# selau642/QuantizedAttention

Measured on AMD Instinct MI355X. Metric: fused-attn fwd+bwd TFLOP/s & us/call at (B,H,S,D)=(4,32,4096,128), int8 vs bf16, higher is better.
Workload: dtype int8; 1 GPU; config 3: int8 SageAttention-3 fwd+bwd (4,32,4096,128) per rank, non-causal; global_batch=4, parallelism=batch x head shard over 1 GPU(s)

## Files before the change

### quantizedattention_amd/csrc/int8_bwd.hip

```cpp
#include <climits>
#include <type_traits>
#include <cstdlib>

#include "tile_image.h"

namespace qattn {

template <int D>
struct I8BwdCfg {
  static constexpr int NKS8 = D / 32;
  static constexpr int NDB = D / 32;
  static constexpr int T8 = I8Rows<D>::TILE;
  static constexpr int T16 = B16Tr<D>::TILE;
};

QA_DEVICE void quant_operand(const float* x, float inv, float c, v8bf* out) {
#pragma unroll
  for (int s = 0; s < 2; ++s) {
    v4u w;
#pragma unroll
    for (int j = 0; j < 4; ++j) {
      const int i0 = 8 * s + 2 * j;
      w[j] = pk_bf16(__builtin_truncf(x[i0] * inv) * c, __builtin_truncf(x[i0 + 1] * inv) * c);
    }
    out[s] = __builtin_bit_cast(v8bf, w);
  }
}

#ifndef QA_PREP_HOIST
#define QA_PREP_HOIST 1
#endif
template <int D, bool IMG>
__global__ __launch_bounds__(256) void int8_bwd_prep_kernel(
    const _Float16* __restrict__ dO, const _Float16* __restrict__ O, const _Float16* __restrict__ lse,
    int8_t* __restrict__ idx, _Float16* __restrict__ scale, __bf16* __restrict__ img,
    float2* __restrict__ LD, long nblocks) {
  constexpr int ELEMS = 32 * D;
  constexpr int ITERS = ELEMS / 512;
  constexpr int TPR = D / 8;
  const int lane = threadIdx.x & 63;
  const long blk = (long)blockIdx.x * 4 + (threadIdx.x >> 6);
  if (blk >= nblocks) return;
  const _Float16* xb = dO + blk * ELEMS;
  const _Float16* ob = O + blk * ELEMS;
  v8h v[ITERS];
  float amax = 0.f;
#if QA_PREP_HOIST
  v8h ov[ITERS];
  _Float16 lsev[ITERS];
#pragma unroll
  for (int i = 0; i < ITERS; ++i) {
    const int e = (i * 64 + lane) * 8;
    v[i] = *reinterpret_cast<const v8h*>(xb + e);
    ov[i] = *reinterpret_cast<const v8h*>(ob + e);
    lsev[i] = lse[blk * 32 + e / D];
  }
#endif
#pragma unroll
  for (int i = 0; i < ITERS; ++i) {
    const int e = (i * 64 + lane) * 8;
#if QA_PREP_HOIST
    const v8h o = ov[i];
#else
    v[i] = *reinterpret_cast<const v8h*>(xb + e);
    const v8h o = *reinterpret_cast<const v8h*>(ob + e);
#endif
    float dsum = 0.f;
#pragma unroll
    for (int j = 0; j < 8; ++j) {
      amax = fmaxf(amax, fabsf((float)v[i][j]));
      dsum += (float)(_Float16)((float)v[i][j] * (float)o[j]);
    }
#pragma unroll
    for (int m = TPR / 2; m >= 1; m >>= 1) dsum += __shfl_xor(dsum, m);
    if (lane % TPR == 0) {
      const long row = blk * 32 + e / D;
#if QA_PREP_HOIST
      LD[row] = float2{(float)lsev[i], (float)(_Float16)dsum};
#else
      LD[row] = float2{(float)lse[row], (float)(_Float16)dsum};
#endif
    }
  }
  amax = wave_max_f(amax);
  const _Float16 s16 = (_Float16)(amax / 127.0f);
  const float s = (float)s16;
  const float r = quant_rcp(s);
  if (lane == 0) scale[blk] = s16;
#pragma unroll
  for (int i = 0; i < ITERS; ++i) {
    const int e = (i * 64 + lane) * 8;
    unsigned lo, hi;
    float qf[8];
    quant8(v[i], s, r, lo, hi, qf);
    *reinterpret_cast<v2u*>(idx + blk * ELEMS + e) = v2u{lo, hi};
    if constexpr (IMG) {
      const v4u w = {pk_bf16(qf[0], qf[1]), pk_bf16(qf[2], qf[3]), pk_bf16(qf[4], qf[5]),
                     pk_bf16(qf[6], qf[7])};
      *reinterpret_cast<v4u*>(img + blk * ELEMS + e) = w;
    }
  }
}
__global__ __launch_bounds__(256) void i8_to_bf16_kernel(const int8_t* __restrict__ x,
                                                         __bf16* __restrict__ y, long n16) {
  const long i = (long)blockIdx.x * 256 + threadIdx.x;
  if (i >= n16) return;
  const v4i w = reinterpret_cast<const v4i*>(x)[i];
  v4u lo, hi;
#pragma unroll
  for (int k = 0; k < 4; ++k) {
    unsigned p[2];
#pragma unroll
    for (int j = 0; j < 2; ++j) {
      const float a = (float)((w[k] << (24 - 16 * j)) >> 24);
      const float b = (float)((w[k] << (16 - 16 * j)) >> 24);
      p[j] = (__float_as_uint(a) >> 16) | (__float_as_uint(b) & 0xffff0000u);
    }
    if (k < 2) { lo[2 * k] = p[0]; lo[2 * k + 1] = p[1]; }
    else { hi[2 * k - 4] = p[0]; hi[2 * k - 3] = p[1]; }
  }
  reinterpret_cast<v4u*>(y)[2 * i] = lo;
  reinterpret_cast<v4u*>(y)[2 * i + 1] = hi;
}

enum BwdRole { ROLE_DV = 0, ROLE_DK = 1, ROLE_DQ = 2, ROLE_DKV = 3 };
#ifndef QA_DKV_PIPE
#define QA_DKV_PIPE 0
#endif
#ifndef QA_DKV_STAGGER
#define QA_DKV_STAGGER 1
#endif
#ifndef QA_DKV_I8DV_COST
#define QA_DKV_I8DV_COST 0
#endif
#ifndef QA_DKV_WAVES
#define QA_DKV_WAVES 8
#endif
#ifndef QA_DKV_NSLOT
#define QA_DKV_NSLOT 4
#endif
#ifndef QA_DKV_HG
#define QA_DKV_HG 4
#endif
#ifndef QA_DQW_HG
#define QA_DQW_HG 0
#endif
#ifndef QA_DKV_PRIO
#define QA_DKV_PRIO 0
#endif
#ifndef QA_DQW_PRIO
#define QA_DQW_PRIO 0
#endif
#ifndef QA_BWD_PACK_ASM
#define QA_BWD_PACK_ASM 1
#endif


template <int D, int ROLE>
struct BwdCfg {
  using C = I8BwdCfg<D>;
  static constexpr bool TWO = ROLE != ROLE_DV;
  static constexpr bool HAS_LD = ROLE != ROLE_DQ;
  static constexpr bool WANT_P = ROLE == ROLE_DV || ROLE == ROLE_DKV;
  static constexpr bool WANT_DS = ROLE != ROLE_DV;
  static constexpr int NTR = (ROLE == ROLE_DKV) ? 2 : 1;
  static constexpr int WAVES = (ROLE == ROLE_DKV) ? QA_DKV_WAVES : 4;
  static constexpr bool PIPE = ROLE != ROLE_DKV;
  static constexpr int Y8A = 0;
  static constexpr int Y8B = C::T8;
  static constexpr int TR = TWO ? 2 * C::T8 : C::T8;
  static constexpr int TR2 = TR + C::T16;
  static constexpr int LDO = TR + NTR * C::T16;
  static constexpr int SLOT = LDO + (HAS_LD ? 256 : 0);
  static constexpr int NSLOT = (ROLE == ROLE_DKV) ? QA_DKV_NSLOT : 4;
  static constexpr int NP8 = I8Rows<D>::NP, NP16 = B16Tr<D>::NP;
  static constexpr int INST = NP8 * (TWO ? 2 : 1) + NTR * NP16;
  static constexpr int IPW16 = (INST + WAVES - 1) / WAVES;
  static constexpr int IPW = IPW16 + (HAS_LD ? 1 : 0);
  static constexpr int XROWS = 32 * WAVES;
};

template <int D, typename G>
struct BwdDmaT {
  unsigned voff[G::IPW16];
  unsigned lds_off[G::IPW16];
  unsigned stride[G::IPW16];
  v4u rsrc[G::IPW16];
  v4u ld_rsrc;
  QA_DEVICE void init(int wave, int lane, int S, const char* y8a, const char* y8b, const char* tr,
                      const char* tr2, const char* ld) {
#pragma unroll
    for (int i = 0; i < G::IPW16; ++i) {
      int p = wave + G::WAVES * i;
      if (p >= G::INST) p = wave;
      if (p < G::NP8) {
        set_i8(i, G::Y8A, p, lane);
        rsrc[i] = make_rsrc(y8a, (unsigned)S * D);
      } else if (G::TWO && p < 2 * G::NP8) {
        set_i8(i, G::Y8B, p - G::NP8, lane);
        rsrc[i] = make_rsrc(y8b, (unsigned)S * D);
      } else {
        int q = p - (G::TWO ? 2 : 1) * G::NP8;
        const bool second = q >= G::NP16;
        if (second) q -= G::NP16;
        voff[i] = B16Tr<D>::dma_src(q, lane);
        lds_off[i] = (second ? G::TR2 : G::TR) + q * 1024;
        stride[i] = B16Tr<D>::TILE;
        rsrc[i] = make_rsrc(second ? tr2 : tr, (unsigned)S * 2 * D);
      }
    }
    if constexpr (G::HAS_LD) ld_rsrc = make_rsrc(ld, (unsigned)S * 8);
  }
  QA_DEVICE void set_i8(int i, int region, int piece, int lane) {
    voff[i] = I8Rows<D>::dma_src(piece, lane);
    lds_off[i] = region + piece * 1024;
    stride[i] = I8Rows<D>::TILE;
  }
  QA_DEVICE void issue(unsigned slot_lds, int t, int lane) const {
#pragma unroll
    for (int i = 0; i < G::IPW16; ++i)
      dma16_buf(rsrc[i], voff[i], (unsigned)t * stride[i], slot_lds + lds_off[i]);
    if constexpr (G::HAS_LD) dma4_buf(ld_rsrc, 4 * lane, (unsigned)t * 256, slot_lds + G::LDO);
  }
};
template <int D, int ROLE>
using BwdDma = BwdDmaT<D, BwdCfg<D, ROLE>>;


QA_DEVICE void floor_magic16(float* y, float inv) {
  const float magic = 8388608.0f;
  asm("s_setreg_imm32_b32 hwreg(HW_REG_MODE, 0, 2), 3\n\t"
      "s_nop 1\n\t"
      "v_fma_f32 %0, %0, %16, %17\n\tv_fma_f32 %1, %1, %16, %17\n\t"
      "v_fma_f32 %2, %2, %16, %17\n\tv_fma_f32 %3, %3, %16, %17\n\t"
      "v_fma_f32 %4, %4, %16, %17\n\tv_fma_f32 %5, %5, %16, %17\n\t"
      "v_fma_f32 %6, %6, %16, %17\n\tv_fma_f32 %7, %7, %16, %17\n\t"
      "v_fma_f32 %8, %8, %16, %17\n\tv_fma_f32 %9, %9, %16, %17\n\t"
      "v_fma_f32 %10, %10, %16, %17\n\tv_fma_f32 %11, %11, %16, %17\n\t"
      "v_fma_f32 %12, %12, %16, %17\n\tv_fma_f32 %13, %13, %16, %17\n\t"
      "v_fma_f32 %14, %14, %16, %17\n\tv_fma_f32 %15, %15, %16, %17\n\t"
      "s_setreg_imm32_b32 hwreg(HW_REG_MODE, 0, 2), 0\n\t"
      "s_nop 1"
      : "+v"(y[0]), "+v"(y[1]), "+v"(y[2]), "+v"(y[3]), "+v"(y[4]), "+v"(y[5]), "+v"(y[6]),
        "+v"(y[7]), "+v"(y[8]), "+v"(y[9]), "+v"(y[10]), "+v"(y[11]), "+v"(y[12]), "+v"(y[13]),
        "+v"(y[14]), "+v"(y[15])
      : "v"(inv), "s"(magic));
}

QA_DEVICE v4i pack16_i8(const float* x) {
  float r0 = x[0], r1 = x[4], r2 = x[8], r3 = x[12];
#define QA_SDWA(R, A, B, U) \
  "v_cvt_i32_f32_sdwa " R ", " A " dst_sel:BYTE_" B " dst_unused:UNUSED_" U " src0_sel:DWORD\n\t"
  asm(QA_SDWA("%0", "%0", "0", "PAD") QA_SDWA("%1", "%1", "0", "PAD")
      QA_SDWA("%2", "%2", "0", "PAD") QA_SDWA("%3", "%3", "0", "PAD")
      QA_SDWA("%0", "%4", "1", "PRESERVE") QA_SDWA("%1", "%7", "1", "PRESERVE")
      QA_SDWA("%2", "%10", "1", "PRESERVE") QA_SDWA("%3", "%13", "1", "PRESERVE")
      QA_SDWA("%0", "%5", "2", "PRESERVE") QA_SDWA("%1", "%8", "2", "PRESERVE")
      QA_SDWA("%2", "%11", "2", "PRESERVE") QA_SDWA("%3", "%14", "2", "PRESERVE")
      QA_SDWA("%0", "%6", "3", "PRESERVE") QA_SDWA("%1", "%9", "3", "PRESERVE")
      QA_SDWA("%2", "%12", "3", "PRESERVE") QA_SDWA("%3", "%15", "3", "PRESERVE")
      : "+v"(r0), "+v"(r1), "+v"(r2), "+v"(r3)
      : "v"(x[1]), "v"(x[2]), "v"(x[3]), "v"(x[5]), "v"(x[6]), "v"(x[7]), "v"(x[9]), "v"(x[10]),
        "v"(x[11]), "v"(x[13]), "v"(x[14]), "v"(x[15]));
#undef QA_SDWA
  return v4i{__float_as_int(r0), __float_as_int(r1), __float_as_int(r2), __float_as_int(r3)};
}

QA_DEVICE float max16_abs3(const float* x) {
  float m = fmaxf(fmaxf(fabsf(x[0]), fabsf(x[1])), fabsf(x[2]));
#pragma unroll
  for (int i = 3; i < 15; i += 2) m = fmaxf(fmaxf(m, fabsf(x[i])), fabsf(x[i + 1]));
  return fmaxf(m, fabsf(x[15]));
}

template <int D>
QA_DEVICE void store_acc_row(const v16f* acc, float sc, _Float16* dst, const long& row, const int& h) {
#pragma unroll
  for (int b = 0; b < D / 32; ++b) {
#pragma unroll
    for (int g = 0; g < 4; ++g) {
      v4h w;
#pragma unroll
      for (int j = 0; j < 4; ++j) w[j] = (_Float16)(acc[b][4 * g + j] * sc);
      *reinterpret_cast<v4h*>(dst + row * D + 32 * b + 8 * g + 4 * h) = w;
    }
  }
}

#ifndef QA_DKV_STAMP
#define QA_DKV_STAMP 0
#endif
#if QA_DKV_STAMP
__device__ unsigned long long g_dkv_stamp[4096][4];
#define DKV_STAMP(k)                                                                            \
  do {                                                                                          \
    if (ROLE == ROLE_DKV && WS && threadIdx.x == 0 && blockIdx.x < 4096)                         \
      g_dkv_stamp[blockIdx.x][k] = __builtin_amdgcn_s_memrealtime();                            \
  } while (0)
#else
#define DKV_STAMP(k) do { } while (0)
#endif
template <int D, int ROLE, bool CAUSAL = false, bool WS = false>
__global__ __launch_bounds__((64 * BwdCfg<D, ROLE>::WAVES), (8 / BwdCfg<D, ROLE>::WAVES))
void int8_bwd_kernel(
    const int8_t* __restrict__ x8a, const int8_t* __restrict__ x8b, const _Float16* __restrict__ sxa,
    const _Float16* __restrict__ sxb, const int8_t* __restrict__ y8a, const int8_t* __restrict__ y8b,
    const __bf16* __restrict__ ytr, const __bf16* __restrict__ ytr2, const float2* __restrict__ yld,
    const _Float16* __restrict__ sya, const _Float16* __restrict__ syb,
    const float2* __restrict__ xld, _Float16* __restrict__ out, _Float16* __restrict__ out2, int BH,
    int Sx, int Ny, int ydiv, int Smod, float qks, float sms, int8_t* __restrict__ ds8,
    float* __restrict__ sds) {
  using C = I8BwdCfg<D>;
  using G = BwdCfg<D, ROLE>;
  constexpr bool TWO = G::TWO;
  static_assert(!WS || ROLE == ROLE_DKV, "the dS workspace is written by the fused dK+dV kernel");
  DKV_STAMP(0);
  extern __shared__ __attribute__((aligned(16))) char smem[];
  const int nxb = (Sx + G::XROWS - 1) / G::XROWS;
  int bh, xt;
  if constexpr (CAUSAL && ROLE == ROLE_DKV && QA_DKV_HG > 0)
    xcd_remap_lpt_grouped(blockIdx.x, nxb, BH, false, QA_DKV_HG, bh, xt);
  else if constexpr (CAUSAL) xcd_remap_lpt(blockIdx.x, nxb, BH, ROLE == ROLE_DQ, bh, xt);
  else xcd_remap(blockIdx.x, nxb, BH, bh, xt);
  const int tid = threadIdx.x;
  const int wave = __builtin_amdgcn_readfirstlane(tid >> 6);
  const int lane = tid & 63, h = lane >> 5, c32 = lane & 31;
  const int x0 = xt * G::XROWS + wave * 32;
  const bool active = x0 < Sx;
  const long hrow = (long)bh * Sx;
  const long yrow = (long)(bh / ydiv) * Ny;
  const int nt = (CAUSAL && ROLE == ROLE_DQ) ? min(Ny / 32, (xt * G::XROWS + G::XROWS) / 32) : Ny / 32;
  const int t0 = (CAUSAL && ROLE != ROLE_DQ && Ny == Smod) ? min(nt, (xt * G::XROWS) / 32) : 0;

  BwdDma<D, ROLE> dma;
  dma.init(wave, lane, Ny, reinterpret_cast<const char*>(y8a + yrow * D),
           reinterpret_cast<const char*>(y8b + yrow * D), reinterpret_cast<const char*>(ytr + yrow * D),
           reinterpret_cast<const char*>(ytr2 + yrow * D), reinterpret_cast<const char*>(yld + yrow));
  const unsigned smem_lds = lds_addr(smem);
#pragma unroll
  for (int i = 0; i < G::NSLOT - 1; ++i)
    dma.issue(smem_lds + ((t0 + i) % G::NSLOT) * G::SLOT, min(t0 + i, nt - 1), lane);
  _Float16* sc_lds = reinterpret_cast<_Float16*>(smem + G::NSLOT * G::SLOT);
  for (int i = tid; i < nt; i += 64 * G::WAVES) {
    sc_lds[i] = sya[yrow / 32 + i];
    sc_lds[nt + i] = syb[yrow / 32 + i];
  }

  v4i xa[C::NKS8], xb[C::NKS8];
  float sxaw = 0.f, sxbw = 0.f, lsex = 0.f, Dx = 0.f;
  if (active) {
    const long r = hrow + x0 + c32;
#pragma unroll
    for (int s = 0; s < C::NKS8; ++s) {
      xa[s] = *reinterpret_cast<const v4i*>(x8a + r * D + 16 * h + 32 * s);
      if constexpr (TWO) xb[s] = *reinterpret_cast<const v4i*>(x8b + r * D + 16 * h + 32 * s);
    }
    sxaw = (float)sxa[(hrow + x0) / 32];
    sxbw = (float)sxb[(hrow + x0) / 32];
    if constexpr (!G::HAS_LD) {
      const float2 v = xld[r];
      lsex = v.x;
      Dx = v.y;
    }
  }
  int roff[C::NKS8], troff[C::NDB];
#pragma unroll
  for (int s = 0; s < C::NKS8; ++s) roff[s] = I8Rows<D>::row_off(c32, 2 * s + h);
  const auto trl = B16Tr<D>::tr_lane(lane, h);
#pragma unroll
  for (int b = 0; b < C::NDB; ++b) troff[b] = B16Tr<D>::tr_off(trl, b);
  v16f acc[C::NDB], acc2[ROLE == ROLE_DKV ? C::NDB : 1];
#pragma unroll
  for (int b = 0; b < C::NDB; ++b) acc[b] = v16f{};
  if constexpr (ROLE == ROLE_DKV) {
#pragma unroll
    for (int b = 0; b < C::NDB; ++b) acc2[b] = v16f{};
  }

  auto slot = [&](int t) -> const char* { return smem + (t % G::NSLOT) * G::SLOT; };
  auto products = [&](int t, v16i& sa, v16i& pa) {
    const char* base = slot(t);
    sa = v16i{};
    pa = v16i{};
#pragma unroll
    for (int s = 0; s < C::NKS8; ++s) {
      sa = mfma_i8(*reinterpret_cast<const v4i*>(base + G::Y8A + roff[s]), xa[s], sa);
      if constexpr (TWO) pa = mfma_i8(*reinterpret_cast<const v4i*>(base + G::Y8B + roff[s]), xb[s], pa);
    }
  };
  auto values = [&](int t, const v16i& sa, const v16i& pa, float* P, float* dS, auto maskc) {
    constexpr bool MASK = CAUSAL && decltype(maskc)::value;
    const int y0 = (32 * t) % Smod;
    const bool diag = MASK && (ROLE == ROLE_DQ ? (y0 + 31 > x0) : (x0 + 31 > y0));
    const float sy_a = (float)sc_lds[t], sy_b = (float)sc_lds[nt + t];
    float c1, c2;
    if constexpr (ROLE == ROLE_DQ) {
      c1 = sxaw * (sy_a * qks);
      c2 = sxbw * sy_b;
    } else {
      c1 = sy_a * (sxaw * qks);
      c2 = sy_b * sxbw;
    }
    const int ln = __lane_id();
    const int lane_rel = (ln & 31) - 4 * (ln >> 5);
    const int dd = !diag ? INT_MIN
                         : (ROLE == ROLE_DQ ? (y0 - x0) - lane_rel : (x0 - y0) + lane_rel);
    if constexpr (G::HAS_LD) {
      const float* ld = reinterpret_cast<const float*>(slot(t) + G::LDO);
#pragma unroll
      for (int g = 0; g < 4; ++g) {
        const v4f a = *reinterpret_cast<const v4f*>(ld + 2 * (8 * g + 4 * h));
        const v4f b = *reinterpret_cast<const v4f*>(ld + 2 * (8 * g + 4 * h) + 4);
        const float lse_r[4] = {a[0], a[2], b[0], b[2]};
        const float d_r[4] = {a[1], a[3], b[1], b[3]};
#pragma unroll
        for (int j = 0; j < 4; ++j) {
          const int i = 4 * g + j;
          float p = exp2_f32(fmaf((float)sa[i], c1, -lse_r[j]));
          if (MASK && dd > 8 * g + j) p = 0.f;
          if constexpr (G::WANT_P) P[i] = p;
          if constexpr (G::WANT_DS) dS[i] = p * fmaf((float)pa[i], c2, -d_r[j]);
        }
      }
    } else {
#pragma unroll
      for (int i = 0; i < 16; ++i) {
        float p = exp2_f32(fmaf((float)sa[i], c1, -lsex));
        if (MASK && dd > -((i & 3) + 8 * (i >> 2))) p = 0.f;
        dS[i] = p * fmaf((float)pa[i], c2, -Dx);
      }
    }
  };
  auto quantise_m = [&](const float* X, float so, v8bf* op, float xmax) {
    const float sx = xmax * (1.0f / 127.0f);
    const float inv = xmax > 0.f ? 127.0f * __builtin_amdgcn_rcpf(xmax) : 0.f;
    quant_operand(X, inv, sx * so, op);
  };
  auto quantise = [&](const float* X, float so, v8bf* op) {
    quantise_m(X, so, op, wave_max_nonneg(max16_abs3(X)));
  };
  auto quantise_p = [&](const float* X, float so, v8bf* op, float xmax) {
    const float sx = xmax * (1.0f / 127.0f);
    const float inv = xmax > 0.f ? 127.0f * __builtin_amdgcn_rcpf(xmax) : 0.f;
    const float c = sx * so;
    const float nc = -8388608.0f * c;
    float y[16];
#if QA_BWD_PACK_ASM
#pragma unroll
    for (int i = 0; i < 16; ++i) y[i] = X[i];
    floor_magic16(y, inv);
#else
#pragma unroll
    for (int i = 0; i < 16; ++i) y[i] = __builtin_truncf(X[i] * inv) + 8388608.0f;
#endif
#pragma unroll
    for (int s = 0; s < 2; ++s) {
      v4u w;
#pragma unroll
      for (int j = 0; j < 4; ++j) {
        const int i0 = 8 * s + 2 * j;
        w[j] = pk_bf16(fmaf(y[i0], c, nc), fmaf(y[i0 + 1], c, nc));
      }
      op[s] = __builtin_bit_cast(v8bf, w);
    }
  };
  auto tr_load = [&](int t, int region, v8bf* ta) { B16Tr<D>::tr_load(slot(t) + region, troff, ta); };
  auto accumulate_i8cost = [&](v16f* ac, const v8bf* ta, const v8bf* op, float c) {
    v16i seed;
#pragma unroll
    for (int i = 0; i < 16; ++i) seed[i] = KMAG_BITS;
#pragma unroll
    for (int b = 0; b < C::NDB; ++b) {
      const v16i pacc = mfma_i8(__builtin_bit_cast(v4i, ta[b]), __builtin_bit_cast(v4i, op[0]), seed);
#pragma unroll
      for (int r = 0; r < 16; ++r) ac[b][r] = fmaf(__int_as_float(pacc[r]), c, ac[b][r]);
    }
  };
  auto accumulate = [&](v16f* ac, const v8bf* ta, const v8bf* op) {
#pragma unroll
    for (int s = 0; s < 2; ++s)
#pragma unroll
      for (int b = 0; b < C::NDB; ++b) ac[b] = mfma_bf16(ta[s * C::NDB + b], op[s], ac[b]);
  };
  auto so_p = [&](int t) { return (float)sc_lds[nt + t]; };
  auto so_ds = [&](int t) { return (float)sc_lds[t]; };
  const long ws_first = WS ? (long)bh * (Ny / 32) * (Sx / 32) : 0;
  const int ws_nrec = WS ? (Ny / 32) * (Sx / 32) : 0;
  const __amdgpu_buffer_rsrc_t ws_rsrc =
      __builtin_amdgcn_make_buffer_rsrc(ds8 + ws_first * 1024, 0, ws_nrec * 1024, 0x00020000);
  float* sds_lds = reinterpret_cast<float*>(smem + G::NSLOT * G::SLOT +
                                            ((2 * nt * 2 + 15) / 16) * 16);
  auto quantise_ds = [&](const float* X, int t, v8bf* op, float xmax) {
    if constexpr (!WS) {
      quantise_m(X, so_ds(t), op, xmax);
    } else {
      const float sx = xmax * (1.0f / 127.0f);
      const float inv = xmax > 0.f ? 127.0f * __builtin_amdgcn_rcpf(xmax) : 0.f;
      const float c = sx * so_ds(t);
      float q[16];
#pragma unroll
      for (int i = 0; i < 16; ++i) q[i] = __builtin_truncf(X[i] * inv);
#pragma unroll
      for (int s = 0; s < 2; ++s) {
        v4u w;
#pragma unroll
        for (int j = 0; j < 4; ++j) w[j] = pk_bf16(q[8 * s + 2 * j] * c, q[8 * s + 2 * j + 1] * c);
        op[s] = __builtin_bit_cast(v8bf, w);
      }
#if QA_BWD_PACK_ASM
      const v4i bytes = pack16_i8(q);
#else
      v4i bytes;
#pragma unroll
      for (int d = 0; d < 4; ++d) {
        const unsigned lo = __builtin_amdgcn_perm((unsigned)(int)q[4 * d + 1], (unsigned)(int)q[4 * d],
                                                  0x0c0c0400u);
        const unsigned hi = __builtin_amdgcn_perm((unsigned)(int)q[4 * d + 3], (unsigned)(int)q[4 * d + 2],
                                                  0x0c0c0400u);
        bytes[d] = (int)__builtin_amdgcn_perm(hi, lo, 0x05040100u);
      }
#endif
      const int nqt = Smod / 32, nkt = Sx / 32;
      const unsigned rel = (unsigned)(t * nkt + x0 / 32);
      __builtin_amdgcn_raw_buffer_store_b128(__builtin_bit_cast(v4u, bytes), ws_rsrc,
                                             16 * (lane ^ ((lane >> 5) << 2)) + (int)(rel * 1024u), 0, 0);
      (void)nqt;
      if (lane == 0) sds_lds[wave * nt + t] = sx;
    }
  };
  constexpr int WS_OPS = WS ? 1 : 0;

  vmem_drain();
  __syncthreads();
  DKV_STAMP(1);
  if constexpr (G::PIPE) {
    float X[16];
    if (active && t0 < nt) {
      v16i sa, pa;
      products(t0, sa, pa);
      values(t0, sa, pa, X, X, std::true_type{});
    }
    for (int t = t0; t < nt; ++t) {
      ring_wait_barrier<(G::NSLOT - 3) * G::IPW>();
      dma.issue(smem_lds + ((t + G::NSLOT - 1) % G::NSLOT) * G::SLOT,
                min(t + G::NSLOT - 1, nt - 1), lane);
      if (active) {
        const int tn = min(t + 1, nt - 1);
        v8bf ta[2 * C::NDB];
        tr_load(t, G::TR, ta);
        v16i sa, pa;
        products(tn, sa, pa);
        v8bf op[2];
        if constexpr (ROLE == ROLE_DV) quantise_p(X, so_p(t), op, wave_max_nonneg(max16_abs3(X)));
        else quantise(X, so_ds(t), op);
        accumulate(acc, ta, op);
        values(tn, sa, pa, X, X, std::true_type{});
      }
    }
  } else {
    const int tb = !CAUSAL ? t0 : (Ny == Smod ? min(nt, t0 + G::WAVES) : nt);
    if (QA_DKV_PRIO == 1 && wave >= G::WAVES / 2) __builtin_amdgcn_s_setprio(1);
    if (QA_DKV_PRIO == 2 && wave < G::WAVES / 2) __builtin_amdgcn_s_setprio(1);
    if (QA_DKV_PIPE || (QA_DKV_STAGGER && wave >= G::WAVES / 2)) {
      v8bf opS[2], opP[2];
      if (active && t0 < nt) {
        v16i sa, pa;
        products(t0, sa, pa);
        float P[16], dS[16];
        values(t0, sa, pa, P, dS, std::true_type{});
        float mS = max16_abs3(dS), mP = max16_abs3(P);
        wave_max2_nonneg(mS, mP);
        quantise_ds(dS, t0, opS, mS);
        quantise_p(P, so_p(t0), opP, mP);
      }
      auto iter = [&](int t, auto maskc) {
        if (active) ring_wait_barrier<(G::NSLOT - 3) * G::IPW + 2 * WS_OPS>();
        else ring_wait_barrier<(G::NSLOT - 3) * G::IPW>();
        dma.issue(smem_lds + ((t + G::NSLOT - 1) % G::NSLOT) * G::SLOT,
                  min(t + G::NSLOT - 1, nt - 1), lane);
        if (active) {
          const int tn = min(t + 1, nt - 1);
          v16i sa, pa;
          products(tn, sa, pa);
          v8bf ta[2 * C::NDB];
          tr_load(t, G::TR, ta);
          accumulate(acc, ta, opS);
          tr_load(t, G::TR2, ta);
#if QA_DKV_I8DV_COST
          accumulate_i8cost(acc2, ta, opP, so_p(t));
#else
          accumulate(acc2, ta, opP);
#endif
          float P[16], dS[16];
          values(tn, sa, pa, P, dS, maskc);
          float mS = max16_abs3(dS), mP = max16_abs3(P);
          wave_max2_nonneg(mS, mP);
          quantise_ds(dS, tn, opS, mS);
          quantise_p(P, so_p(tn), opP, mP);
        }
      };
      int t = t0;
      for (; t < tb; ++t) iter(t, std::true_type{});
      for (; t < nt; ++t) iter(t, std::false_type{});
    } else {
      auto iter = [&](int t, auto maskc) {
        if (active)
          ring_wait_barrier<(G::NSLOT - (QA_DKV_STAGGER ? 3 : 2)) * G::IPW +
                            (QA_DKV_STAGGER ? 2 : 3) * WS_OPS>();
        else
          ring_wait_barrier<(G::NSLOT - (QA_DKV_STAGGER ? 3 : 2)) * G::IPW>();
        dma.issue(smem_lds + ((t + G::NSLOT - 1) % G::NSLOT) * G::SLOT,
                  min(t + G::NSLOT - 1, nt - 1), lane);
        if (active) {
          v16i sa, pa;
          products(t, sa, pa);
          float P[16], dS[16];
          values(t, sa, pa, P, dS, maskc);
          v8bf opS[2], opP[2];
          float mS = max16_abs3(dS), mP = max16_abs3(P);
          wave_max2_nonneg(mS, mP);
          quantise_ds(dS, t, opS, mS);
          quantise_p(P, so_p(t), opP, mP);
          v8bf ta[2 * C::NDB];
          tr_load(t, G::TR, ta);
          accumulate(acc, ta, opS);
          tr_load(t, G::TR2, ta);
#if QA_DKV_I8DV_COST
          accumulate_i8cost(acc2, ta, opP, so_p(t));
#else
          accumulate(acc2, ta, opP);
#endif
        }
      };
      int t = t0;
      for (; t < tb; ++t) iter(t, std::true_type{});
      for (; t < nt; ++t) iter(t, std::false_type{});
    }
  }
  vmcnt_wait_all();
  DKV_STAMP(2);
  if (!active) return;
  if constexpr (WS) {
    const int nkt = Sx / 32;
    for (int t = t0 + lane; t < nt; t += 64) sds[ws_first + (long)t * nkt + x0 / 32] = sds_lds[wave * nt + t];
  }
  const long r = hrow + x0 + c32;
  store_acc_row<D>(acc, ROLE == ROLE_DV ? 1.0f : sms, out, r, h);
  if constexpr (ROLE == ROLE_DKV) store_acc_row<D>(acc2, 1.0f, out2, r, h);
#if QA_DKV_STAMP
  asm volatile("s_waitcnt vmcnt(0)" ::: "memory");
  DKV_STAMP(3);
#endif
}


#ifndef QA_DQW_WAVES
#define QA_DQW_WAVES 8
#endif
#ifndef QA_DQW_DIAG
#define QA_DQW_DIAG 0
#endif
#ifndef QA_DQW_NT
#define QA_DQW_NT 1
#endif
#ifndef QA_DQW_TR8
#define QA_DQW_TR8 0
#endif
#ifndef QA_DQW_NSLOT
#define QA_DQW_NSLOT 4
#endif
#ifndef QA_DQW_ALLOW_WIDE
static_assert(QA_DQW_WAVES <= 8, "dQ-from-records workgroups may not exceed the dK+dV kernel's 8 waves");
#endif
template <int D>
struct DqwCfg {
  static constexpr int WAVES = QA_DQW_WAVES;
  static constexpr int T16 = B16Tr<D>::TILE;
  static constexpr int NSLOT = QA_DQW_NSLOT;
#ifdef QA_DQW_RSLOT
  static constexpr int RSLOT = QA_DQW_RSLOT;
#else
  static constexpr int RSLOT = WAVES >= 16 ? 4 : WAVES == 8 ? 5 : 10;
#endif
  static constexpr int REC = WAVES * 1024;
  static constexpr int RBASE = NSLOT * T16;
  static constexpr int IPK = TrImageDma<D, WAVES>::IPK;
  static_assert(RSLOT - 1 >= NSLOT, "record ring must run ahead of the k image ring");
};

template <int D, bool CAUSAL>
__global__ __launch_bounds__(64 * QA_DQW_WAVES, QA_DQW_WAVES >= 16 ? 4 : 2) void int8_bwd_dqw_kernel(
    const int8_t* __restrict__ ds8, const float* __restrict__ sds, const __bf16* __restrict__ kbf,
    const _Float16* __restrict__ sk, _Float16* __restrict__ dq, int BH, int Sq, int Sk, int G,
    float sms) {
  using C = I8BwdCfg<D>;
  using W = DqwCfg<D>;
  extern __shared__ __attribute__((aligned(16))) char smem[];
  const int nqb = (Sq + 32 * W::WAVES - 1) / (32 * W::WAVES);
  int bh, qb;
  if constexpr (CAUSAL && QA_DQW_HG > 0) xcd_remap_lpt_grouped(blockIdx.x, nqb, BH, true, QA_DQW_HG, bh, qb);
  else if constexpr (CAUSAL) xcd_remap_lpt(blockIdx.x, nqb, BH, true, bh, qb);
  else xcd_remap(blockIdx.x, nqb, BH, bh, qb);
  const int tid = threadIdx.x;
  const int wave = __builtin_amdgcn_readfirstlane(tid >> 6);
  const int lane = tid & 63, h = lane >> 5, c32 = lane & 31;
  const int q0 = qb * 32 * W::WAVES + wave * 32;
  const bool active = q0 < Sq;
  const int nqt = Sq / 32, nkt = Sk / 32;
  const long kv_row0 = (long)(bh / G) * Sk;
  const int nt = CAUSAL ? min(nkt, (qb * 32 * W::WAVES + 32 * W::WAVES) / 32) : nkt;
  const long rec0 = ((long)bh * nqt + (active ? q0 / 32 : 0)) * nkt;

  TrImageDma<D, W::WAVES> kdma;
  kdma.init(wave, lane, kbf + kv_row0 * D, (unsigned)Sk);
  const v4u rrsrc = make_rsrc(ds8 + rec0 * 1024, active ? (unsigned)nkt * 1024u : 0u);
  const unsigned smem_lds = lds_addr(smem);
  auto issue_k = [&](int t) {
    if (!(QA_DQW_DIAG & 8))
      kdma.issue(smem_lds + (t % W::NSLOT) * W::T16, (QA_DQW_DIAG & 2) ? 0u : (unsigned)min(t, nt - 1) * W::T16);
  };
  auto issue_r = [&](int t, int rs) {
    if (QA_DQW_DIAG & 4) return;
#if QA_DQW_NT
    dma16_buf_nt(rrsrc, 16u * lane, (QA_DQW_DIAG & 1) ? 0u : (unsigned)min(t, nt - 1) * 1024u,
#else
    dma16_buf(rrsrc, 16u * lane, (QA_DQW_DIAG & 1) ? 0u : (unsigned)min(t, nt - 1) * 1024u,
#endif
              smem_lds + W::RBASE + rs * W::REC + wave * 1024);
  };
#pragma unroll
  for (int i = 0; i < W::NSLOT - 1; ++i) issue_k(i);
#pragma unroll
  for (int i = 0; i < W::RSLOT - 1; ++i) issue_r(i, i);
  float* c_lds = reinterpret_cast<float*>(smem + W::RBASE + W::RSLOT * W::REC);
  for (int i = lane; i < nt; i += 64) c_lds[wave * nkt + i] = active ? sds[rec0 + i] * (float)sk[kv_row0 / 32 + i] : 0.f;

#if QA_DQW_TR8
  int rtr;
  {
    const int j = (lane & 15) >> 1;
    const int hq = (lane >> 4) & 1;
    rtr = 16 * (((8 * (j >> 2) + 4 * h + (j & 3)) ^ (4 * hq)) + 32 * hq) + 8 * (lane & 1);
  }
#else
  v4i perm = {0, 0, 0, 0};
  if (((c32 >> 2) & 1) == h) {
    const int i = 4 * (c32 >> 3) + (c32 & 3);
    perm[i >> 2] = 1 << (8 * (i & 3));
  }
#endif
  int troff[C::NDB];
  const auto trl = B16Tr<D>::tr_lane(lane, h);
#pragma unroll
  for (int b = 0; b < C::NDB; ++b) troff[b] = B16Tr<D>::tr_off(trl, b);
  v16f acc[C::NDB];
#pragma unroll
  for (int b = 0; b < C::NDB; ++b) acc[b] = v16f{};

  auto make_op = [&](int t, int rs, v8bf* op) {
    const float c = c_lds[wave * nkt + t];
#if QA_DQW_TR8
    const char* rb = smem + W::RBASE + rs * W::REC + wave * 1024 + rtr;
#pragma unroll
    for (int s = 0; s < 2; ++s) {
      const v2i x = __builtin_amdgcn_ds_read_tr8_b64_v2i32(
          (__attribute__((address_space(3))) v2i*)(rb + 256 * s));
      v4u w;
#pragma unroll
      for (int j = 0; j < 4; ++j) {
        const int wd = x[j >> 1], sh = 16 * (j & 1);
        w[j] = pk_bf16((float)(signed char)(wd >> sh) * c, (float)(signed char)(wd >> (sh + 8)) * c);
      }
      op[s] = __builtin_bit_cast(v8bf, w);
    }
#else
    const v4i rec = *reinterpret_cast<const v4i*>(smem + W::RBASE + rs * W::REC + wave * 1024 +
                                                  16 * (lane ^ ((lane >> 5) << 2)));
    const v16i x = mfma_i8(rec, perm, v16i{});
#pragma unroll
    for (int s = 0; s < 2; ++s) {
      v4u w;
#pragma unroll
      for (int j = 0; j < 4; ++j)
        w[j] = pk_bf16((float)x[8 * s + 2 * j] * c, (float)x[8 * s + 2 * j + 1] * c);
      op[s] = __builtin_bit_cast(v8bf, w);
    }
#endif
  };

  vmem_drain();
  __syncthreads();
  v8bf op[2];
  make_op(0, 0, op);
  if (QA_DQW_PRIO && wave >= W::WAVES / 2) __builtin_amdgcn_s_setprio(1);
  auto step = [&](int t, int rs_next, int rs_issue) {
    ring_wait_barrier<(W::RSLOT - 1 > W::NSLOT ? 1 : 0) + (W::NSLOT - 2) * (W::IPK + 1)>();
    issue_k(t + W::NSLOT - 1);
    issue_r(t + W::RSLOT - 1, rs_issue);
    v8bf ta[2 * C::NDB];
    B16Tr<D>::tr_load(smem + (t % W::NSLOT) * W::T16, troff, ta);
    v8bf opn[2];
    make_op(t + 1, rs_next, opn);
#pragma unroll
    for (int s = 0; s < 2; ++s)
#pragma unroll
      for (int b = 0; b < C::NDB; ++b) acc[b] = mfma_bf16(ta[s * C::NDB + b], op[s], acc[b]);
    op[0] = opn[0];
    op[1] = opn[1];
  };
  int t = 0;
  for (; t + W::RSLOT <= nt; t += W::RSLOT) {
    static_for<W::RSLOT>([&](auto J) {
      constexpr int j = decltype(J)::value;
      step(t + j, (j + 1) % W::RSLOT, (j + W::RSLOT - 1) % W::RSLOT);
    });
  }
  for (; t < nt; ++t) step(t, (t + 1) % W::RSLOT, (t + W::RSLOT - 1) % W::RSLOT);
  vmcnt_wait_all();
  if (!active) return;
#if QA_DQW_TR8
  const long r = (long)bh * Sq + q0 + 8 * ((c32 & 15) >> 2) + 4 * (c32 >> 4) + (c32 & 3);
#else
  const long r = (long)bh * Sq + q0 + c32;
#endif
  store_acc_row<D>(acc, sms, dq, r, h);
}

}

using namespace qattn;

extern "C" int qattn_int8_bwd_prep(const void* dO, const void* O, const void* lse, void* dO_i8,
                                   void* sdO, void* LD, void* dO_bf, long bh, long seq, int head_dim,
                                   void* stream) {
  if (seq % 32 != 0 || (head_dim != 64 && head_dim != 128)) return 1;
  const long nblocks = bh * seq / 32;
  if (nblocks == 0) return 0;
  dim3 grid((unsigned)((nblocks + 3) / 4)), block(256);
  hipStream_t st = (hipStream_t)stream;
#define QA_LAUNCH(Dv, IM)                                                                       \
  hipLaunchKernelGGL((int8_bwd_prep_kernel<Dv, IM>), grid, block, 0, st, (const _Float16*)dO,   \
                     (const _Float16*)O, (const _Float16*)lse, (int8_t*)dO_i8, (_Float16*)sdO,   \
                     (__bf16*)dO_bf, (float2*)LD, nblocks)
  if (head_dim == 128) {
    if (dO_bf) QA_LAUNCH(128, true); else QA_LAUNCH(128, false);
  } else {
    if (dO_bf) QA_LAUNCH(64, true); else QA_LAUNCH(64, false);
  }
#undef QA_LAUNCH
  return hipGetLastError() == hipSuccess ? 0 : 2;
}

extern "C" int qattn_i8_to_bf16(const void* x, void* y, long n, void* stream) {
  if (n % 16 != 0) return 1;
  const long n16 = n / 16;
  if (n16 == 0) return 0;
  hipLaunchKernelGGL(i8_to_bf16_kernel, dim3((unsigned)((n16 + 255) / 256)), dim3(256), 0,
                     (hipStream_t)stream, (const int8_t*)x, (__bf16*)y, n16);
  return hipGetLastError() == hipSuccess ? 0 : 2;
}

struct BwdArgs {
  const void *dO_i8, *sdO, *q_i8, *sq, *k_i8, *sk, *v_i8, *sv, *LD, *q_bf, *k_bf, *dO_bf;
  void *dq, *dk, *dv;
  long bh, sqt, skt;
  int group, causal, head_dim;
  float qks, sms;
  void* stream;
  void* ws = nullptr;
  char* ds8() const { return (char*)ws; }
  char* sds() const { return (char*)ws + bh * (sqt / 32) * (skt / 32) * 1024; }
};

template <int D, int ROLE, bool CAUSAL, bool WS>
static void launch_bwd_c(const BwdArgs& a) {
  using G = BwdCfg<D, ROLE>;
  constexpr bool DQ = ROLE == ROLE_DQ, DV = ROLE == ROLE_DV, DKV = ROLE == ROLE_DKV;
  const long bhx = DQ ? a.bh : a.bh / a.group, sx = DQ ? a.sqt : a.skt;
  const long ny = DQ ? a.skt : a.group * a.sqt, smod = DQ ? a.skt : a.sqt;
  const int lds = G::NSLOT * G::SLOT + (int)((2 * (ny / 32) * 2 + 15) / 16 * 16) +
                  (WS ? G::WAVES * (int)(ny / 32) * 4 : 0);
  { static LdsGrant granted_; lds_grant((const void*)int8_bwd_kernel<D, ROLE, CAUSAL, WS>, lds, granted_); }
  const int nb = (int)((sx + G::XROWS - 1) / G::XROWS);
  hipLaunchKernelGGL(
      (int8_bwd_kernel<D, ROLE, CAUSAL, WS>), dim3((unsigned)(nb * bhx)), dim3(64 * G::WAVES), lds,
      (hipStream_t)a.stream,
      (const int8_t*)(DQ ? a.q_i8 : a.k_i8), (const int8_t*)(DQ ? a.dO_i8 : DV ? nullptr : a.v_i8),
      (const _Float16*)(DQ ? a.sq : a.sk), (const _Float16*)(DQ ? a.sdO : a.sv),
      (const int8_t*)(DQ ? a.k_i8 : a.q_i8), (const int8_t*)(DQ ? a.v_i8 : DV ? nullptr : a.dO_i8),
      (const __bf16*)(DQ ? a.k_bf : DV ? a.dO_bf : a.q_bf), (const __bf16*)(DKV ? a.dO_bf : nullptr),
      (const float2*)(DQ ? nullptr : a.LD), (const _Float16*)(DQ ? a.sk : a.sq),
      (const _Float16*)(DQ ? a.sv : a.sdO), (const float2*)(DQ ? a.LD : nullptr),
      (_Float16*)(DQ ? a.dq : DV ? a.dv : a.dk), (_Float16*)(DKV ? a.dv : nullptr), (int)bhx, (int)sx,
      (int)ny, DQ ? a.group : 1, (int)smod, a.qks, a.sms, (int8_t*)(WS ? a.ds8() : nullptr),
      (float*)(WS ? a.sds() : nullptr));
}
template <int D, int ROLE, bool WS = false>
static void launch_bwd(const BwdArgs& a) {
  if (a.causal) launch_bwd_c<D, ROLE, true, WS>(a);
  else launch_bwd_c<D, ROLE, false, WS>(a);
}

template <int D, bool CAUSAL>
static void launch_dqw_c(const BwdArgs& a) {
  using G = DqwCfg<D>;
  const int nkt = (int)(a.skt / 32);
  const int lds = G::RBASE + G::RSLOT * G::REC + G::WAVES * nkt * 4 + 16;
  { static LdsGrant granted_; lds_grant((const void*)int8_bwd_dqw_kernel<D, CAUSAL>, lds, granted_); }
  const int nb = (int)((a.sqt + 32 * G::WAVES - 1) / (32 * G::WAVES));
  hipLaunchKernelGGL((int8_bwd_dqw_kernel<D, CAUSAL>), dim3((unsigned)(nb * a.bh)),
                     dim3(64 * G::WAVES), lds, (hipStream_t)a.stream, (const int8_t*)a.ds8(),
                     (const float*)a.sds(), (const __bf16*)a.k_bf, (const _Float16*)a.sk,
                     (_Float16*)a.dq, (int)a.bh, (int)a.sqt, (int)a.skt, a.group, a.sms);
}

template <int D>
static void bwd_launch_d(int which, const BwdArgs& a) {
  if (which & 16) launch_bwd<D, ROLE_DKV, true>(a);
  if (which & 32) {
    if (a.causal) launch_dqw_c<D, true>(a);
    else launch_dqw_c<D, false>(a);
  }
  if (which & 1) launch_bwd<D, ROLE_DV>(a);
  if (which & 4) launch_bwd<D, ROLE_DK>(a);
  if (which & 8) launch_bwd<D, ROLE_DKV>(a);
  if (which & 2) launch_bwd<D, ROLE_DQ>(a);
}

static int int8_bwd_launch(int which, const BwdArgs& a) {
  if (a.sqt % 32 != 0 || a.skt % 32 != 0 || a.group < 1 || a.bh % a.group != 0 ||
      (a.head_dim != 64 && a.head_dim != 128))
    return 1;
  if (a.bh == 0 || a.sqt == 0) return 0;
  if (a.skt == 0) return 1;
  if (a.head_dim == 128) bwd_launch_d<128>(which, a);
  else bwd_launch_d<64>(which, a);
  return hipGetLastError() == hipSuccess ? 0 : 2;
}

// ... 125 lines not shown
```

Measured before the change: 994.9 TFLOP/s.

## Use region-major LDS ring and unroll dKV loop by slot count for non-causal

For the non-causal fused dK+dV kernel, the LDS ring is reorganised from slot-major to region-major: each of the int8 tiles, the LSE/D rows and the transposed bf16 tiles gets its own contiguous group of slots. The main loop is then unrolled by NSLOT using compile-time slot indices, so LDS addresses become a base register plus a constant offset. This is meant to remove per-iteration modulo and address arithmetic and to let ds_read immediate offsets be used. The costs are more code, higher register pressure, and a static_assert-limited layout that requires every region group to fit in a 16-bit offset window.

```diff
diff --git a/quantizedattention_amd/csrc/int8_bwd.hip b/quantizedattention_amd/csrc/int8_bwd.hip
--- a/quantizedattention_amd/csrc/int8_bwd.hip
+++ b/quantizedattention_amd/csrc/int8_bwd.hip
@@ -139,6 +139,9 @@
 #ifndef QA_DKV_NSLOT
 #define QA_DKV_NSLOT 4
 #endif
+#ifndef QA_DKV_UNROLL
+#define QA_DKV_UNROLL 1
+#endif
 #ifndef QA_DKV_HG
 #define QA_DKV_HG 4
 #endif
@@ -156,7 +159,7 @@
 #endif
 
 
-template <int D, int ROLE>
+template <int D, int ROLE, bool BYR = false>
 struct BwdCfg {
   using C = I8BwdCfg<D>;
   static constexpr bool TWO = ROLE != ROLE_DV;
@@ -178,6 +181,17 @@
   static constexpr int IPW16 = (INST + WAVES - 1) / WAVES;
   static constexpr int IPW = IPW16 + (HAS_LD ? 1 : 0);
   static constexpr int XROWS = 32 * WAVES;
+  static constexpr bool BY_REGION = BYR;
+  static_assert(!BYR || ROLE == ROLE_DKV, "only the fused dK+dV kernel has the region-major ring");
+  static constexpr int I8_STRIDE = BY_REGION ? 2 * C::T8 : SLOT;
+  static constexpr int LD_STRIDE = BY_REGION ? 256 : SLOT;
+  static constexpr int TR_STRIDE = BY_REGION ? NTR * C::T16 : SLOT;
+  static constexpr int I8_BASE = 0;
+  static constexpr int LD_BASE = BY_REGION ? NSLOT * I8_STRIDE : LDO;
+  static constexpr int TR_BASE = BY_REGION ? LD_BASE + NSLOT * LD_STRIDE : TR;
+  static_assert(!BY_REGION || (TR_BASE + NSLOT * TR_STRIDE == NSLOT * SLOT && LD_BASE + NSLOT * LD_STRIDE < 65536 &&
+                               NSLOT * TR_STRIDE <= 65536),
+                "region-major ring: same size, every region group inside one 16-bit offset window");
 };
 
 template <int D, typename G>
@@ -187,6 +201,7 @@
   unsigned stride[G::IPW16];
   v4u rsrc[G::IPW16];
   v4u ld_rsrc;
+  unsigned lds_str[G::BY_REGION ? G::IPW16 : 1];
   QA_DEVICE void init(int wave, int lane, int S, const char* y8a, const char* y8b, const char* tr,
                       const char* tr2, const char* ld) {
 #pragma unroll
@@ -204,16 +219,26 @@
         const bool second = q >= G::NP16;
         if (second) q -= G::NP16;
         voff[i] = B16Tr<D>::dma_src(q, lane);
-        lds_off[i] = (second ? G::TR2 : G::TR) + q * 1024;
+        lds_off[i] = (G::BY_REGION ? G::TR_BASE + (second ? G::C::T16 : 0) : second ? G::TR2 : G::TR) + q * 1024;
+        if constexpr (G::BY_REGION) lds_str[i] = G::TR_STRIDE;
         stride[i] = B16Tr<D>::TILE;
         rsrc[i] = make_rsrc(second ? tr2 : tr, (unsigned)S * 2 * D);
       }
     }
     if constexpr (G::HAS_LD) ld_rsrc = make_rsrc(ld, (unsigned)S * 8);
+    if constexpr (G::BY_REGION) {
+#pragma unroll
+      for (int i = 0; i < G::IPW16; ++i) {
+        lds_off[i] = __builtin_amdgcn_readfirstlane(lds_off[i]);
+        lds_str[i] = __builtin_amdgcn_readfirstlane(lds_str[i]);
+        stride[i] = __builtin_amdgcn_readfirstlane(stride[i]);
+      }
+    }
   }
   QA_DEVICE void set_i8(int i, int region, int piece, int lane) {
     voff[i] = I8Rows<D>::dma_src(piece, lane);
     lds_off[i] = region + piece * 1024;
+    if constexpr (G::BY_REGION) lds_str[i] = G::I8_STRIDE;
     stride[i] = I8Rows<D>::TILE;
   }
   QA_DEVICE void issue(unsigned slot_lds, int t, int lane) const {
@@ -221,6 +246,16 @@
     for (int i = 0; i < G::IPW16; ++i)
       dma16_buf(rsrc[i], voff[i], (unsigned)t * stride[i], slot_lds + lds_off[i]);
     if constexpr (G::HAS_LD) dma4_buf(ld_rsrc, 4 * lane, (unsigned)t * 256, slot_lds + G::LDO);
+  }
+  QA_DEVICE void issue_slot(unsigned ring_lds, int s, int t, int lane) const {
+    if constexpr (!G::BY_REGION) {
+      issue(ring_lds + s * G::SLOT, t, lane);
+    } else {
+#pragma unroll
+      for (int i = 0; i < G::IPW16; ++i)
+        dma16_buf(rsrc[i], voff[i], (unsigned)t * stride[i], ring_lds + lds_off[i] + s * lds_str[i]);
+      dma4_buf(ld_rsrc, 4 * lane, (unsigned)t * 256, ring_lds + G::LD_BASE + s * G::LD_STRIDE);
+    }
   }
 };
 template <int D, int ROLE>
@@ -311,7 +346,7 @@
     int Sx, int Ny, int ydiv, int Smod, float qks, float sms, int8_t* __restrict__ ds8,
     float* __restrict__ sds) {
   using C = I8BwdCfg<D>;
-  using G = BwdCfg<D, ROLE>;
+  using G = BwdCfg<D, ROLE, ROLE == ROLE_DKV && QA_DKV_UNROLL && !CAUSAL>;
   constexpr bool TWO = G::TWO;
   static_assert(!WS || ROLE == ROLE_DKV, "the dS workspace is written by the fused dK+dV kernel");
   DKV_STAMP(0);
@@ -332,14 +367,14 @@
   const int nt = (CAUSAL && ROLE == ROLE_DQ) ? min(Ny / 32, (xt * G::XROWS + G::XROWS) / 32) : Ny / 32;
   const int t0 = (CAUSAL && ROLE != ROLE_DQ && Ny == Smod) ? min(nt, (xt * G::XROWS) / 32) : 0;
 
-  BwdDma<D, ROLE> dma;
+  BwdDmaT<D, G> dma;
   dma.init(wave, lane, Ny, reinterpret_cast<const char*>(y8a + yrow * D),
            reinterpret_cast<const char*>(y8b + yrow * D), reinterpret_cast<const char*>(ytr + yrow * D),
            reinterpret_cast<const char*>(ytr2 + yrow * D), reinterpret_cast<const char*>(yld + yrow));
   const unsigned smem_lds = lds_addr(smem);
 #pragma unroll
   for (int i = 0; i < G::NSLOT - 1; ++i)
-    dma.issue(smem_lds + ((t0 + i) % G::NSLOT) * G::SLOT, min(t0 + i, nt - 1), lane);
+    dma.issue_slot(smem_lds, (t0 + i) % G::NSLOT, min(t0 + i, nt - 1), lane);
   _Float16* sc_lds = reinterpret_cast<_Float16*>(smem + G::NSLOT * G::SLOT);
   for (int i = tid; i < nt; i += 64 * G::WAVES) {
     sc_lds[i] = sya[yrow / 32 + i];
@@ -388,11 +423,12 @@
       if constexpr (TWO) pa = mfma_i8(*reinterpret_cast<const v4i*>(base + G::Y8B + roff[s]), xb[s], pa);
     }
   };
-  auto values = [&](int t, const v16i& sa, const v16i& pa, float* P, float* dS, auto maskc) {
+  auto values_at = [&](int t, auto sya_of, auto syb_of, auto ld_of, const v16i& sa, const v16i& pa,
+                       float* P, float* dS, auto maskc) {
     constexpr bool MASK = CAUSAL && decltype(maskc)::value;
     const int y0 = (32 * t) % Smod;
     const bool diag = MASK && (ROLE == ROLE_DQ ? (y0 + 31 > x0) : (x0 + 31 > y0));
-    const float sy_a = (float)sc_lds[t], sy_b = (float)sc_lds[nt + t];
+    const float sy_a = sya_of(), sy_b = syb_of();
     float c1, c2;
     if constexpr (ROLE == ROLE_DQ) {
       c1 = sxaw * (sy_a * qks);
@@ -406,11 +442,11 @@
     const int dd = !diag ? INT_MIN
                          : (ROLE == ROLE_DQ ? (y0 - x0) - lane_rel : (x0 - y0) + lane_rel);
     if constexpr (G::HAS_LD) {
-      const float* ld = reinterpret_cast<const float*>(slot(t) + G::LDO);
 #pragma unroll
       for (int g = 0; g < 4; ++g) {
-        const v4f a = *reinterpret_cast<const v4f*>(ld + 2 * (8 * g + 4 * h));
-        const v4f b = *reinterpret_cast<const v4f*>(ld + 2 * (8 * g + 4 * h) + 4);
+        const float* ld = ld_of(g);
+        const v4f a = *reinterpret_cast<const v4f*>(ld);
+        const v4f b = *reinterpret_cast<const v4f*>(ld + 4);
         const float lse_r[4] = {a[0], a[2], b[0], b[2]};
         const float d_r[4] = {a[1], a[3], b[1], b[3]};
 #pragma unroll
@@ -430,6 +466,11 @@
         dS[i] = p * fmaf((float)pa[i], c2, -Dx);
       }
     }
+  };
+  auto values = [&](int t, const v16i& sa, const v16i& pa, float* P, float* dS, auto maskc) {
+    values_at(t, [&] { return (float)sc_lds[t]; }, [&] { return (float)sc_lds[nt + t]; },
+              [&](int g) { return reinterpret_cast<const float*>(slot(t) + G::LDO) + 2 * (8 * g + 4 * h); },
+              sa, pa, P, dS, maskc);
   };
   auto quantise_m = [&](const float* X, float so, v8bf* op, float xmax) {
     const float sx = xmax * (1.0f / 127.0f);
@@ -490,13 +531,13 @@
       __builtin_amdgcn_make_buffer_rsrc(ds8 + ws_first * 1024, 0, ws_nrec * 1024, 0x00020000);
   float* sds_lds = reinterpret_cast<float*>(smem + G::NSLOT * G::SLOT +
                                             ((2 * nt * 2 + 15) / 16) * 16);
-  auto quantise_ds = [&](const float* X, int t, v8bf* op, float xmax) {
+  auto quantise_ds_at = [&](const float* X, int t, auto so_of, v8bf* op, float xmax) {
     if constexpr (!WS) {
-      quantise_m(X, so_ds(t), op, xmax);
+      quantise_m(X, so_of(), op, xmax);
     } else {
       const float sx = xmax * (1.0f / 127.0f);
       const float inv = xmax > 0.f ? 127.0f * __builtin_amdgcn_rcpf(xmax) : 0.f;
-      const float c = sx * so_ds(t);
+      const float c = sx * so_of();
       float q[16];
 #pragma unroll
       for (int i = 0; i < 16; ++i) q[i] = __builtin_truncf(X[i] * inv);
@@ -527,6 +568,9 @@
       (void)nqt;
       if (lane == 0) sds_lds[wave * nt + t] = sx;
     }
+  };
+  auto quantise_ds = [&](const float* X, int t, v8bf* op, float xmax) {
+    quantise_ds_at(X, t, [&] { return so_ds(t); }, op, xmax);
   };
   constexpr int WS_OPS = WS ? 1 : 0;
 
@@ -561,8 +605,105 @@
     const int tb = !CAUSAL ? t0 : (Ny == Smod ? min(nt, t0 + G::WAVES) : nt);
     if (QA_DKV_PRIO == 1 && wave >= G::WAVES / 2) __builtin_amdgcn_s_setprio(1);
     if (QA_DKV_PRIO == 2 && wave < G::WAVES / 2) __builtin_amdgcn_s_setprio(1);
+    using DynSlot = std::integral_constant<int, -1>;
+    auto ring = [&](int t, auto SL, int ahead) -> int {
+      constexpr int s = decltype(SL)::value;
+      if constexpr (s < 0) return (t + ahead) % G::NSLOT;
+      else return (s + ahead) % G::NSLOT;
+    };
+    auto issue_ahead = [&](int t, auto SL) {
+      dma.issue_slot(smem_lds, ring(t, SL, G::NSLOT - 1), min(t + G::NSLOT - 1, nt - 1), lane);
+    };
+    unsigned rp[C::NKS8], tp[C::NDB], lp = smem_lds + G::LD_BASE + 32 * h;
+#pragma unroll
+    for (int k = 0; k < C::NKS8; ++k) {
+      rp[k] = smem_lds + G::I8_BASE + roff[k];
+      asm("" : "+v"(rp[k]));
+    }
+#pragma unroll
+    for (int b = 0; b < C::NDB; ++b) {
+      tp[b] = smem_lds + G::TR_BASE + troff[b];
+      asm("" : "+v"(tp[b]));
+    }
+    auto lds_at = [](unsigned a) -> const char* {
+      return (const char*)(__attribute__((address_space(3))) const char*)(uintptr_t)a;
+    };
+    auto products_u = [&](int s, v16i& sa, v16i& pa) {
+      sa = v16i{};
+      pa = v16i{};
+#pragma unroll
+      for (int k = 0; k < C::NKS8; ++k) {
+        const char* a = lds_at(rp[k] + s * G::I8_STRIDE);
+        sa = mfma_i8(*reinterpret_cast<const v4i*>(a), xa[k], sa);
+        pa = mfma_i8(*reinterpret_cast<const v4i*>(a + C::T8), xb[k], pa);
+      }
+    };
+    auto values_u = [&](int t, int s, float sy_a, float sy_b, const v16i& sa, const v16i& pa, float* P,
+                        float* dS, auto maskc) {
+      values_at(t, [&] { return sy_a; }, [&] { return sy_b; },
+                [&](int g) { return reinterpret_cast<const float*>(lds_at(lp + s * G::LD_STRIDE + 64 * g)); },
+                sa, pa, P, dS, maskc);
+    };
+    auto tr_load_u = [&](int s, int image, v8bf* ta) {
+      static_assert(B16Tr<D>::period(16), "rows r and r + 16 must share an offset");
+#pragma unroll
+      for (int r = 0; r < 2; ++r)
+#pragma unroll
+        for (int b = 0; b < C::NDB; ++b)
+          ta[r * C::NDB + b] = B16Tr<D>::tr_frag(lds_at(tp[b] + s * G::TR_STRIDE + image * C::T16 +
+                                                        16 * r * B16Tr<D>::ROWB));
+    };
+    auto tiles = [&](auto iter, int tend) {
+      int t = t0;
+      for (; t < tb; ++t) iter(t, DynSlot{}, std::true_type{});
+      for (; t % G::NSLOT == 0 && t + G::NSLOT <= tend; t += G::NSLOT)
+        static_for<G::NSLOT>([&](auto J) { iter(t + decltype(J)::value, J, std::false_type{}); });
+      for (; t < nt; ++t) iter(t, DynSlot{}, std::false_type{});
+    };
     if (QA_DKV_PIPE || (QA_DKV_STAGGER && wave >= G::WAVES / 2)) {
       v8bf opS[2], opP[2];
+      if constexpr (G::BY_REGION) {
+      if (active && t0 < nt) {
+        const float sq_0 = (float)sc_lds[t0], sdo_0 = (float)sc_lds[nt + t0];
+        v16i sa, pa;
+        products_u(t0 % G::NSLOT, sa, pa);
+        float P[16], dS[16];
+        values_u(t0, t0 % G::NSLOT, sq_0, sdo_0, sa, pa, P, dS, std::true_type{});
+        float mS = max16_abs3(dS), mP = max16_abs3(P);
+        wave_max2_nonneg(mS, mP);
+        quantise_ds_at(dS, t0, [&] { return sq_0; }, opS, mS);
+        quantise_p(P, sdo_0, opP, mP);
+      }
+      auto iter = [&](int t, auto SL, auto maskc) {
+        constexpr bool DYN = decltype(SL)::value < 0;
+        if (active) ring_wait_barrier<(G::NSLOT - 3) * G::IPW + 2 * WS_OPS>();
+        else ring_wait_barrier<(G::NSLOT - 3) * G::IPW>();
+        issue_ahead(t, SL);
+        if (active) {
+          const int tn = DYN ? min(t + 1, nt - 1) : t + 1;
+          const int st = ring(t, SL, 0), sn = DYN ? tn % G::NSLOT : ring(t, SL, 1);
+          v16i sa, pa;
+          products_u(sn, sa, pa);
+          v8bf ta[2 * C::NDB];
+          tr_load_u(st, 0, ta);
+          accumulate(acc, ta, opS);
+          tr_load_u(st, 1, ta);
+#if QA_DKV_I8DV_COST
+          accumulate_i8cost(acc2, ta, opP, so_p(t));
+#else
+          accumulate(acc2, ta, opP);
+#endif
+          const float sq_n = (float)sc_lds[tn], sdo_n = (float)sc_lds[nt + tn];
+          float P[16], dS[16];
+          values_u(tn, sn, sq_n, sdo_n, sa, pa, P, dS, maskc);
+          float mS = max16_abs3(dS), mP = max16_abs3(P);
+          wave_max2_nonneg(mS, mP);
+          quantise_ds_at(dS, tn, [&] { return sq_n; }, opS, mS);
+          quantise_p(P, sdo_n, opP, mP);
+        }
+      };
+      tiles(iter, nt - 1);
+      } else {
       if (active && t0 < nt) {
         v16i sa, pa;
         products(t0, sa, pa);
@@ -602,7 +743,41 @@
       int t = t0;
       for (; t < tb; ++t) iter(t, std::true_type{});
       for (; t < nt; ++t) iter(t, std::false_type{});
+      }
     } else {
+      if constexpr (G::BY_REGION) {
+      auto iter = [&](int t, auto SL, auto maskc) {
+        if (active)
+          ring_wait_barrier<(G::NSLOT - (QA_DKV_STAGGER ? 3 : 2)) * G::IPW +
+                            (QA_DKV_STAGGER ? 2 : 3) * WS_OPS>();
+        else
+          ring_wait_barrier<(G::NSLOT - (QA_DKV_STAGGER ? 3 : 2)) * G::IPW>();
+        issue_ahead(t, SL);
+        if (active) {
+          const int st = ring(t, SL, 0);
+          v16i sa, pa;
+          products_u(st, sa, pa);
+          const float sq_t = (float)sc_lds[t], sdo_t = (float)sc_lds[nt + t];
+          float P[16], dS[16];
+          values_u(t, st, sq_t, sdo_t, sa, pa, P, dS, maskc);
+          v8bf opS[2], opP[2];
+          float mS = max16_abs3(dS), mP = max16_abs3(P);
+          wave_max2_nonneg(mS, mP);
+          quantise_ds_at(dS, t, [&] { return sq_t; }, opS, mS);
+          quantise_p(P, sdo_t, opP, mP);
+          v8bf ta[2 * C::NDB];
+          tr_load_u(st, 0, ta);
+          accumulate(acc, ta, opS);
+          tr_load_u(st, 1, ta);
+#if QA_DKV_I8DV_COST
+          accumulate_i8cost(acc2, ta, opP, sdo_t);
+#else
+          accumulate(acc2, ta, opP);
+#endif
+        }
+      };
+      tiles(iter, nt);
+      } else {
       auto iter = [&](int t, auto maskc) {
         if (active)
           ring_wait_barrier<(G::NSLOT - (QA_DKV_STAGGER ? 3 : 2)) * G::IPW +
@@ -635,6 +810,7 @@
       int t = t0;
       for (; t < tb; ++t) iter(t, std::true_type{});
       for (; t < nt; ++t) iter(t, std::false_type{});
+      }
     }
   }
   vmcnt_wait_all();
```

After: 989.7 TFLOP/s. About the same (-0.5%).
